# TeemoCaption/FDDM-asr

Measured on AMD Instinct MI355X. Metric: train-step utterances/sec (10 s @16 kHz, seq_len 256) at 1/2/4/8 MI355X, higher is better.
Workload: dtype bf16; 1 GPU; fddm_zhTW_base C2: WavLM-base + 6L d512 H8 ff2048 decoder, V=8000, T=200, dropout 0.1, n_step_fd=4; global_batch=32, seq_len=256, parallelism=dp1

## Files before the change

### fddm-asr_amd/csrc/norm.hip

```cpp
#include "common.h"

namespace fddm {

constexpr int LN_MAXPL = 16;

struct LnFwdArgs {
  const void* x; const void* y;
  const float *gamma, *beta, *fsc, *fsh;
  float* out_f32; void* out_t; float* save_s; float *mean, *rstd;
  long N, d, rows_per_batch;
  float eps;
  uint64_t seed, stream; unsigned thr16; float drop_scale;
  const uint64_t* seed_off;
  const float *rcos, *rsin; void* rope_out; long rope_L;
};

template <typename T>
__device__ __forceinline__ void ld8(const T* p, float (&v)[8]) {
  if constexpr (sizeof(T) == 2) {
    const uint4 u = *(const uint4*)p;
    const unsigned w[4] = {u.x, u.y, u.z, u.w};
#pragma unroll
    for (int i = 0; i < 4; ++i) {
      v[2 * i] = __uint_as_float(w[i] << 16);
      v[2 * i + 1] = __uint_as_float(w[i] & 0xffff0000u);
    }
  } else {
    const float4 a = *(const float4*)p, b = *(const float4*)(p + 4);
    v[0] = a.x; v[1] = a.y; v[2] = a.z; v[3] = a.w; v[4] = b.x; v[5] = b.y; v[6] = b.z; v[7] = b.w;
  }
}
template <typename T>
__device__ __forceinline__ void st8(T* p, const float (&v)[8]) {
  if constexpr (sizeof(T) == 2) {
    uint4 u;
    u.x = pk_bf16(v[0], v[1]);
    u.y = pk_bf16(v[2], v[3]);
    u.z = pk_bf16(v[4], v[5]);
    u.w = pk_bf16(v[6], v[7]);
    *(uint4*)p = u;
  } else {
    *(float4*)p = make_float4(v[0], v[1], v[2], v[3]);
    *(float4*)(p + 4) = make_float4(v[4], v[5], v[6], v[7]);
  }
}

template <typename OT>
__device__ __forceinline__ void st4v(OT* p, float a, float b, float c, float d_) {
  if constexpr (sizeof(OT) == 2) {
    *(uint2*)p = make_uint2(pk_bf16(a, b), pk_bf16(c, d_));
  } else {
    *(float4*)p = make_float4(a, b, c, d_);
  }
}

constexpr int LN_MAXCH = 2;

template <int CTRL>
__device__ __forceinline__ float dppf(float v) {
  return __int_as_float(__builtin_amdgcn_update_dpp(0, __float_as_int(v), CTRL, 0xF, 0xF, false));
}
__device__ __forceinline__ float wave_sum_v(float v) {
  v += dppf<0xB1>(v);
  v += dppf<0x4E>(v);
  v += dppf<0x141>(v);
  v += dppf<0x140>(v);
  auto r = __builtin_amdgcn_permlane16_swap(__float_as_uint(v), __float_as_uint(v), false, false);
  v = __uint_as_float(r[0]) + __uint_as_float(r[1]);
  r = __builtin_amdgcn_permlane32_swap(__float_as_uint(v), __float_as_uint(v), false, false);
  return __uint_as_float(r[0]) + __uint_as_float(r[1]);
}

template <typename XT, typename YT, typename OT, bool HY, bool HF, int CH, bool RP = false>
__global__ void __launch_bounds__(256) ln_fwd_kernel(LnFwdArgs a) {
  const int lane = threadIdx.x & 63;
  const long row = (long)blockIdx.x * 4 + __builtin_amdgcn_readfirstlane(threadIdx.x >> 6);
  if (row >= a.N) return;
  const long d = a.d, nch = d / 8;
  const XT* x = (const XT*)a.x + row * d;
  const YT* y = HY ? (const YT*)a.y + row * d : nullptr;
  const long b = HF ? row / a.rows_per_batch : 0;
  float v[CH][8], yv[CH][8], gm[CH][8], bt[CH][8], fs[CH][8], fh[CH][8], rc[CH][8], rs[CH][8];
  const long rp = RP ? row % a.rope_L : 0;
#pragma unroll
  for (int i = 0; i < CH; ++i) {
    const long c0 = min(lane + 64L * i, nch - 1) * 8;
    ld8<XT>(x + c0, v[i]);
    if constexpr (HY) ld8<YT>(y + c0, yv[i]);
    ld8<float>(a.gamma + c0, gm[i]);
    ld8<float>(a.beta + c0, bt[i]);
    if constexpr (HF) {
      ld8<float>(a.fsc + b * d + c0, fs[i]);
      ld8<float>(a.fsh + b * d + c0, fh[i]);
    }
    if constexpr (RP) {
      ld8<float>(a.rcos + rp * d + c0, rc[i]);
      ld8<float>(a.rsin + rp * d + c0, rs[i]);
    }
  }
  float sum = 0.f;
#pragma unroll
  for (int i = 0; i < CH; ++i) {
    const long ch = lane + 64L * i;
    if (ch >= nch) {
#pragma unroll
      for (int e = 0; e < 8; ++e) v[i][e] = 0.f;
    } else {
      if constexpr (HY) {
        unsigned keep = 0xffu;
        if (a.thr16) {
          const uint64_t e4 = (uint64_t)(row * d + ch * 8) >> 2;
          keep = drop_keep4(eff_seed(a.seed, a.seed_off), a.stream, e4, a.thr16) | (drop_keep4(eff_seed(a.seed, a.seed_off), a.stream, e4 + 1, a.thr16) << 4);
        }
#pragma unroll
        for (int e = 0; e < 8; ++e) {
          const float t = yv[i][e];
          v[i][e] += a.thr16 ? ((keep >> e) & 1u ? t * a.drop_scale : 0.f) : t;
        }
      }
#pragma unroll
      for (int e = 0; e < 8; ++e) sum += v[i][e];
    }
  }
  const float mean = wave_sum_v(sum) / (float)d;
  float sq = 0.f;
#pragma unroll
  for (int i = 0; i < CH; ++i) {
    const long ch = lane + 64L * i;
    if (ch < nch) {
#pragma unroll
      for (int e = 0; e < 8; ++e) {
        const float t = v[i][e] - mean;
        sq += t * t;
      }
    }
  }
  const float var = wave_sum_v(sq) / (float)d;
  const float rstd = 1.f / sqrtf(var + a.eps);
#pragma unroll
  for (int i = 0; i < CH; ++i) {
    const long ch = lane + 64L * i;
    if (ch < nch) {
      const long c0 = ch * 8;
      if (a.save_s) st8<float>(a.save_s + row * d + c0, v[i]);
      float o[8];
#pragma unroll
      for (int e = 0; e < 8; ++e) o[e] = (v[i][e] - mean) * rstd * gm[i][e] + bt[i][e];
      if constexpr (HF) {
#pragma unroll
        for (int e = 0; e < 8; ++e) o[e] = o[e] * (1.f + fs[i][e]) + fh[i][e];
      }
      if (a.out_f32) st8<float>(a.out_f32 + row * d + c0, o);
      if (a.out_t) st8<OT>((OT*)a.out_t + row * d + c0, o);
      if constexpr (RP) {
        float lo[4], hi[4];
#pragma unroll
        for (int j = 0; j < 4; ++j) {
          lo[j] = o[2 * j] * rc[i][2 * j] - o[2 * j + 1] * rs[i][2 * j + 1];
          hi[j] = o[2 * j] * rs[i][2 * j] + o[2 * j + 1] * rc[i][2 * j + 1];
        }
        OT* ro = (OT*)a.rope_out + row * d;
        st4v<OT>(ro + 4 * ch, lo[0], lo[1], lo[2], lo[3]);
        st4v<OT>(ro + d / 2 + 4 * ch, hi[0], hi[1], hi[2], hi[3]);
      }
    }
  }
  if (lane == 0) {
    if (a.mean) a.mean[row] = mean;
    if (a.rstd) a.rstd[row] = rstd;
  }
}

struct LnBwdArgs {
  const float* dout; const float* s; const float *mean, *rstd, *gamma, *beta, *fsc;
  float* dres; void* dy_t;
  float *dgamma, *dbeta, *dfsc, *dfsh;
  float* part;
  long N, d, rows_per_batch;
  uint64_t seed, stream; unsigned thr16; float drop_scale;
  const uint64_t* seed_off;
};

template <typename OT>
__global__ void __launch_bounds__(256) ln_bwd_kernel(LnBwdArgs a) {
// ... 300 lines not shown
    if (!(x_dtype == FDDM_F32 && y_dtype == FDDM_BF16 && out_dtype == FDDM_BF16 && hy && !hf))
      return (int)hipErrorInvalidValue;
    if (ch1) hipLaunchKernelGGL((ln_fwd_kernel<float, bf16_t, bf16_t, true, false, 1, true>), grid, dim3(256), 0, s, a);
    else hipLaunchKernelGGL((ln_fwd_kernel<float, bf16_t, bf16_t, true, false, 2, true>), grid, dim3(256), 0, s, a);
    return (int)hipGetLastError();
  }
#define LNF2(XT, YT, OT, C)                                                                                    \
  do {                                                                                                         \
    if (hy && hf) hipLaunchKernelGGL((ln_fwd_kernel<XT, YT, OT, true, true, C>), grid, dim3(256), 0, s, a);     \
    else if (hy) hipLaunchKernelGGL((ln_fwd_kernel<XT, YT, OT, true, false, C>), grid, dim3(256), 0, s, a);     \
    else if (hf) hipLaunchKernelGGL((ln_fwd_kernel<XT, YT, OT, false, true, C>), grid, dim3(256), 0, s, a);     \
    else hipLaunchKernelGGL((ln_fwd_kernel<XT, YT, OT, false, false, C>), grid, dim3(256), 0, s, a);            \
  } while (0)
#define LNF(XT, YT, OT)                \
  do {                                 \
    if (ch1) LNF2(XT, YT, OT, 1);      \
    else LNF2(XT, YT, OT, 2);          \
  } while (0)
  if (x_dtype == FDDM_F32 && y_dtype == FDDM_BF16 && out_dtype == FDDM_BF16)
    LNF(float, bf16_t, bf16_t);
  else if (x_dtype == FDDM_F32 && y_dtype == FDDM_F32 && out_dtype == FDDM_F32)
    LNF(float, float, float);
  else if (x_dtype == FDDM_BF16 && y_dtype == FDDM_BF16 && out_dtype == FDDM_BF16)
    LNF(bf16_t, bf16_t, bf16_t);
  else if (x_dtype == FDDM_F32 && y_dtype == FDDM_F32 && out_dtype == FDDM_BF16)
    LNF(float, float, bf16_t);
  else
    return (int)hipErrorInvalidValue;
#undef LNF
#undef LNF2
  return (int)hipGetLastError();
}

FDDM_API int fddm_ln_bwd(int dy_dtype, const float* dout, const float* s, const float* mean, const float* rstd,
                         const float* gamma, const float* beta, const float* film_scale, float* dres, void* dy_t,
                         float* dgamma, float* dbeta, float* dfilm_scale, float* dfilm_shift, long N, long d,
                         long rows_per_batch, float drop_p, unsigned long long seed, unsigned long long stream,
                         float* partials, void* hs) {
  if (N <= 0) return 0;
  if (d > 64 * LN_MAXPL) return (int)hipErrorInvalidValue;
  if (film_scale && (dgamma || dfilm_scale || dfilm_shift) && !(dfilm_scale && dfilm_shift))
    return (int)hipErrorInvalidValue;
  if ((dgamma == nullptr) != (dbeta == nullptr)) return (int)hipErrorInvalidValue;
  LnBwdArgs a{dout, s, mean, rstd, gamma, beta, film_scale, dres, dy_t, dgamma, dbeta, dfilm_scale, dfilm_shift,
              partials, N, d, rows_per_batch > 0 ? rows_per_batch : N, seed, stream, 0u, 1.f, g_seed_off};
  if (drop_p > 0.f) {
    a.thr16 = (unsigned)llrintf(drop_p * 65536.f);
    a.drop_scale = 1.f / (1.f - drop_p);
  }
  hipStream_t st_ = (hipStream_t)hs;
  const bool vec_ok = d % 8 == 0 && d <= 1024 &&
                      !(((uintptr_t)dout | (uintptr_t)s | (uintptr_t)gamma | (uintptr_t)beta | (uintptr_t)film_scale |
                         (uintptr_t)dres | (uintptr_t)dy_t) & 15);
  const bool fused = (dgamma || dfilm_scale) && (!film_scale || a.rows_per_batch % LNB_ROWS == 0) &&
                     (!dgamma || (beta && dbeta)) && vec_ok;
  if (partials && !dgamma) return (int)hipErrorInvalidValue;
  if (partials && !fused) {
    a.part = nullptr;
    const hipError_t e = hipMemsetAsync(partials, 0, (size_t)((N + LNB_ROWS - 1) / LNB_ROWS) * 4 * d * sizeof(float), st_);
    if (e != hipSuccess) return (int)e;
  }
  if (fused) {
    dim3 fg((unsigned)((N + LNB_ROWS - 1) / LNB_ROWS));
    const bool small = d <= 512;
    if (dy_dtype == FDDM_BF16) {
      if (small) hipLaunchKernelGGL((ln_bwd_fused_kernel<1, bf16_t>), fg, dim3(512), 0, st_, a);
// ... 43 lines not shown
```

### fddm-asr_amd/fddm_hip/functions.py

```python
from __future__ import annotations

import math
import weakref

import torch
import torch.nn.functional as F

from . import ops, runtime as rt

F32 = torch.float32


def _t(x):
    cd = rt.compute_dtype()
    return x if x.dtype == cd else ops.cast(x.contiguous(), cd)


def _gdst(p, zero=False):
    s = rt.grad_slot(p)
    if s is not None:
        return s, True
    return (torch.zeros if zero else torch.empty)(p.shape, device=p.device, dtype=F32), False


# ... 137 lines not shown
            Bt = dtb.shape[0]
            dte = torch.empty(Bt, Wp.shape[1], device=dev, dtype=F32)
            ops.small_linear(dtb, [Wp.detach()], None, [dte], transpose_w=True)
            dpre = torch.empty(Bt, W2.shape[1], device=dev, dtype=F32)
            ops.small_linear(dte, [W2.detach()], None, [dpre], act=2, aux=pre, transpose_w=True)
            ops.small_dw([(dte, h, T[2][0], T[3][0]), (dpre, emb, T[0][0], T[1][0])])
            for i in range(6):
                grads[i] = _ret(*T[i])
        return (None, None, None, None, None) + tuple(grads)


def _film_split(fs):
    return fs.contiguous()


class DecoderBlockFn(torch.autograd.Function):

    @staticmethod
    def forward(ctx, x, xT, cT, key_keep, fscale, fshift, meta, *params):
        (sa_w, sa_b, so_w, so_b, ca_w, ca_b, co_w, co_b, f0_w, f0_b, f3_w, f3_b,
         n1w, n1b, n2w, n2b, n3w, n3b) = params
        B, L, S, H, layer, p, seed, cos, sin = meta[:9]
        N, d = x.shape
        dev = x.device
        cd = rt.compute_dtype()
        st = 6 * layer
        W = {k: rt.wt(v) for k, v in (("sa", sa_w), ("so", so_w), ("ca", ca_w), ("co", co_w), ("f0", f0_w),
                                       ("f3", f3_w))}
        xr = meta[12] if len(meta) > 12 else None
        if xr is None:
            xr = torch.empty(N, d, device=dev, dtype=cd)
            ops.rope_fwd(x, cos, sin, xr, L)
        handoff = meta[13] if len(meta) > 13 else None
        qk = ops.linear(xr, W["sa"][: 2 * d], sa_b[: 2 * d], out_dtype=cd)
        v = ops.linear(xT, W["sa"][2 * d:], sa_b[2 * d:], out_dtype=cd)
        o = torch.empty(N, d, device=dev, dtype=cd)
        lse = torch.empty(B * H, L, device=dev, dtype=F32)
        pre = meta[11] if len(meta) > 11 else None
        ready = pre is not None and p > 0
        bits_s = pre[0] if ready else (ops.drop_bits(B, H, L, L, dev) if p > 0 else None)
        bits_c = pre[1] if ready else (ops.drop_bits(B, H, L, S, dev) if p > 0 else None)
        fwd_s = lambda: ops.attn_fwd(qk, qk[:, d:], v, o, lse, B, H, L, L, key_keep=key_keep, drop_p=p,
                                     seed=seed, rng_stream=st + 1, dbits=bits_s, bits_ready=ready)
        with rt.probe("decoder.self_attn_fwd", replay=fwd_s):
            fwd_s()
        y = ops.linear(o, W["so"], so_b, out_dtype=cd)
        s1 = torch.empty(N, d, device=dev, dtype=F32)
        m1 = torch.empty(N, device=dev, dtype=F32)
        r1 = torch.empty(N, device=dev, dtype=F32)
        x1 = torch.empty(N, d, device=dev, dtype=F32)
        x1T = torch.empty(N, d, device=dev, dtype=cd) if cd != F32 else x1
        ops.ln_fwd(x, y, n1w, n1b, out_f32=x1, out_t=x1T if cd != F32 else None, save_s=s1, mean=m1, rstd=r1,
                   drop_p=p, seed=seed, rng_stream=st + 2)
        qc = ops.linear(x1T, W["ca"][:d], ca_b[:d], out_dtype=cd)
        kvc = meta[10] if len(meta) > 10 and meta[10] is not None else \
            ops.linear(cT, W["ca"][d:], ca_b[d:], out_dtype=cd)
        oc = torch.empty(N, d, device=dev, dtype=cd)
        lsec = torch.empty(B * H, L, device=dev, dtype=F32)
        c_keep = meta[14] if len(meta) > 14 else None
        c_len = meta[15] if len(meta) > 15 else None
        fwd_c = lambda: ops.attn_fwd(qc, kvc, kvc[:, d:], oc, lsec, B, H, L, S, drop_p=p, seed=seed,
                                     rng_stream=st + 3, dbits=bits_c, bits_ready=ready, key_keep=c_keep,
                                     key_len=c_len)
        with rt.probe("decoder.cross_attn_fwd", replay=fwd_c):
            fwd_c()
        yc = ops.linear(oc, W["co"], co_b, out_dtype=cd)
        s2 = torch.empty(N, d, device=dev, dtype=F32)
        m2 = torch.empty(N, device=dev, dtype=F32)
        r2 = torch.empty(N, device=dev, dtype=F32)
        x2 = torch.empty(N, d, device=dev, dtype=F32)
        x2T = torch.empty(N, d, device=dev, dtype=cd) if cd != F32 else x2
        fsc, fsh = fscale.detach().contiguous(), fshift.detach().contiguous()
        ops.ln_fwd(x1, yc, n2w, n2b, out_f32=x2, out_t=x2T if cd != F32 else None, save_s=s2, mean=m2, rstd=r2,
                   film=(fsc, fsh), rows_per_batch=L, drop_p=p, seed=seed, rng_stream=st + 4)
        FF = f0_w.shape[0]
        hpre = torch.empty(N, FF, device=dev, dtype=cd)
        hact = torch.empty(N, FF, device=dev, dtype=cd)
        ops.linear(x2T, W["f0"], f0_b, out=hpre, epi=ops.EPI_GELU, C2=hact, drop_p=p, seed=seed, rng_stream=st + 5)
        y3 = ops.linear(hact, W["f3"], f3_b, out_dtype=cd)
        s3 = torch.empty(N, d, device=dev, dtype=F32)
        m3 = torch.empty(N, device=dev, dtype=F32)
        r3 = torch.empty(N, device=dev, dtype=F32)
        x3 = torch.empty(N, d, device=dev, dtype=F32)
        x3T = torch.empty(N, d, device=dev, dtype=cd)
        rope = None
        if handoff is not None and cd == torch.bfloat16 and d % 16 == 0 and d <= 1024:
            handoff["xr"] = torch.empty(N, d, device=dev, dtype=cd)
            rope = (cos, sin, handoff["xr"], L)
        ops.ln_fwd(x2, y3, n3w, n3b, out_f32=x3, out_t=x3T, save_s=s3, mean=m3, rstd=r3,
                   drop_p=p, seed=seed, rng_stream=st + 6, rope=rope)
        ctx.save_for_backward(xT, xr, qk, v, o, lse, s1, m1, r1, x1T, qc, kvc, oc, lsec, s2, m2, r2, x2T, hpre, hact,
                              s3, m3, r3, cT, key_keep, fsc, *params)
        ctx.meta = meta
        ctx.bits = (bits_s, bits_c)
        ctx.mark_non_differentiable(x3T)
        ctx.set_materialize_grads(False)
        return x3, x3T

    @staticmethod
    def backward(ctx, dx3, _dx3T):
        (xT, xr, qk, v, o, lse, s1, m1, r1, x1T, qc, kvc, oc, lsec, s2, m2, r2, x2T, hpre, hact, s3, m3, r3, cT,
         key_keep, fsc, *params) = ctx.saved_tensors
        (sa_w, sa_b, so_w, so_b, ca_w, ca_b, co_w, co_b, f0_w, f0_b, f3_w, f3_b,
         n1w, n1b, n2w, n2b, n3w, n3b) = params
        B, L, S, H, layer, p, seed, cos, sin = ctx.meta[:9]
        gfilm = ctx.meta[9] if len(ctx.meta) > 9 else None
        st = 6 * layer
        N, d = dx3.shape
        dev = dx3.device
        cd = rt.compute_dtype()
        W = {k: rt.wt(v_) for k, v_ in (("sa", sa_w), ("so", so_w), ("ca", ca_w), ("co", co_w), ("f0", f0_w),
                                         ("f3", f3_w))}
        G = [_gdst(p_, zero=True) for p_ in params]
        (gsa_w, asa), (gsa_b, _), (gso_w, aso), (gso_b, _), (gca_w, aca), (gca_b, _), (gco_w, aco), (gco_b, _), \
            (gf0_w, af0), (gf0_b, _), (gf3_w, af3), (gf3_b, _), (gn1w, _), (gn1b, _), (gn2w, _), (gn2b, _), \
            (gn3w, _), (gn3b, _) = G
        dx3 = dx3.contiguous()
        lnp = ops.LnPartials()
        dx2 = torch.empty(N, d, device=dev, dtype=F32)
        dy3 = torch.empty(N, d, device=dev, dtype=cd)
        ops.ln_bwd(dx3, s3, m3, r3, n3w, n3b, dres=dx2, dy_t=dy3, dgamma=gn3w, dbeta=gn3b, drop_p=p,
                   seed=seed, rng_stream=st + 6, partials=lnp)
        dw_jobs = [(dy3, hact, gf3_w, gf3_b)]
# ... 257 lines not shown
```

### fddm-asr_amd/fddm_hip/ops.py

```python
from __future__ import annotations

import math
import os

import torch

from ._lib import call, lib

F32, BF16 = 0, 1
EPI_STORE, EPI_GELU, EPI_ACC, EPI_GELU_ONLY, EPI_DGELU = 0, 1, 2, 3, 4


def code(t: torch.Tensor) -> int:
    if t.dtype == torch.float32:
        return F32
    if t.dtype == torch.bfloat16:
        return BF16
    raise TypeError(f"unsupported dtype {t.dtype}")


def tdtype(c: int):
    return torch.float32 if c == F32 else torch.bfloat16


# ... 320 lines not shown
def attn_bwd(q, k, v, o, do, lse, dq, dk, dv, B, H, Lq, Lk, *, key_keep=None, drop_p=0.0, seed=0, rng_stream=0,
             dbits=None, scale=None, key_len=None):
    _chk(o.shape[1] % H == 0, "attention output width must be H * head_dim")
    dh = o.shape[1] // H
    _chk(1 <= dh <= 64, f"head_dim {dh} > 64 is not built")
    if key_len is not None:
        _chk_key_len(key_len, key_keep, B, Lk)
    sc = 1.0 / math.sqrt(dh) if scale is None else scale
    if dh != 64:
        rq, rk = B * Lq, B * Lk
        dqp = torch.empty(rq, H * 64, device=dq.device, dtype=dq.dtype)
        dkp = torch.empty(rk, H * 64, device=dk.device, dtype=dk.dtype)
        dvp = torch.empty(rk, H * 64, device=dv.device, dtype=dv.dtype)
        attn_bwd(_pad64(q, rq, H, dh), _pad64(k, rk, H, dh), _pad64(v, rk, H, dh), _pad64(o, rq, H, dh),
                 _pad64(do, rq, H, dh), lse, dqp, dkp, dvp, B, H, Lq, Lk, key_keep=key_keep, drop_p=drop_p, seed=seed,
                 rng_stream=rng_stream, dbits=dbits, scale=sc)
        for g, gp, r in ((dq, dqp, rq), (dk, dkp, rk), (dv, dvp, rk)):
            _heads(g, r, H, dh).copy_(gp.view(r, H, 64)[:, :, :dh])
        return
    delta = torch.empty(int(lib().fddm_attn_bwd_ws_floats(B, H, Lq, Lk)), device=q.device, dtype=torch.float32)
    if key_len is not None:
        call("fddm_attn_bwd_kx", code(q), ptr(q), q.stride(0), ptr(k), k.stride(0), ptr(v), v.stride(0), ptr(o),
             o.stride(0), ptr(do), do.stride(0), ptr(lse), ptr(dq), dq.stride(0), ptr(dk), dk.stride(0), ptr(dv),
             dv.stride(0), ptr(delta), ptr(key_keep), ptr(key_len), B, H, Lq, Lk, float(sc), float(drop_p), seed,
             rng_stream, ptr(dbits), stream())
        return
    call("fddm_attn_bwd", code(q), ptr(q), q.stride(0), ptr(k), k.stride(0), ptr(v), v.stride(0), ptr(o),
         o.stride(0), ptr(do), do.stride(0), ptr(lse), ptr(dq), dq.stride(0), ptr(dk), dk.stride(0), ptr(dv),
         dv.stride(0), ptr(delta), ptr(key_keep), B, H, Lq, Lk, float(sc), float(drop_p), seed, rng_stream,
         ptr(dbits), stream())


def ln_fwd(x, y, gamma, beta, *, out_f32=None, out_t=None, save_s=None, mean=None, rstd=None, film=None,
           rows_per_batch=0, eps=1e-5, drop_p=0.0, seed=0, rng_stream=0, rope=None):
    N, d = x.shape
    fs, fh = film if film is not None else (None, None)
    rc, rs, ro, rl = rope if rope is not None else (None, None, None, 0)
    out_code = code(out_t) if out_t is not None else code(x if y is None else y)
    ycode = code(y) if y is not None else code(x)
    call("fddm_ln_fwd", code(x), ycode, out_code, ptr(x), ptr(y), ptr(gamma), ptr(beta), ptr(fs), ptr(fh),
         ptr(out_f32), ptr(out_t), ptr(save_s), ptr(mean), ptr(rstd), N, d, rows_per_batch, float(eps), float(drop_p),
         seed, rng_stream, ptr(rc), ptr(rs), ptr(ro), rl, stream())


def ln_bwd(dout, s, mean, rstd, gamma, beta, *, dres=None, dy_t=None, dgamma=None, dbeta=None, film_scale=None,
           dfilm=None, rows_per_batch=0, drop_p=0.0, seed=0, rng_stream=0, partials=None):
    N, d = dout.shape
    dfs, dfh = dfilm if dfilm is not None else (None, None)
    part = None
    if partials is not None:
        _chk(dgamma is not None and dbeta is not None, "ln_bwd partials need dgamma and dbeta")
        part = partials.add(N, d, dgamma, dbeta, (dfs, dfh) if film_scale is not None else None, rows_per_batch)
    call("fddm_ln_bwd", code(dy_t) if dy_t is not None else F32, ptr(dout), ptr(s), ptr(mean), ptr(rstd), ptr(gamma),
         ptr(beta), ptr(film_scale), ptr(dres), ptr(dy_t), ptr(dgamma), ptr(dbeta), ptr(dfs), ptr(dfh), N, d,
         rows_per_batch, float(drop_p), seed, rng_stream, ptr(part), stream())


class LnPartials:

    def __init__(self):
        self.jobs = []

    def add(self, N, d, dgamma, dbeta, dfilm=None, rows_per_batch=0):
        _chk(len(self.jobs) < 4, "at most 4 LayerNorms per fold")
        rows = lib().fddm_ln_bwd_slab_rows()
        nslab = (N + rows - 1) // rows
        part = torch.empty(nslab, 4, d, device=dgamma.device, dtype=torch.float32)
        dfs = dfh = None
        spb = 0
        if dfilm is not None and rows_per_batch > 0 and rows_per_batch % rows == 0:
            dfs, dfh = dfilm
            spb = rows_per_batch // rows
        self.jobs.append((part, nslab, d, dgamma, dbeta, dfs, dfh, spb))
        return part

# ... 302 lines not shown
```

### fddm-asr_amd/fddm_hip/runtime.py

```python
from __future__ import annotations

import contextlib
import math
import os

import weakref

import torch

from . import ops

_precision = os.environ.get("FDDM_PRECISION", "bf16")


def precision() -> str:
    return _precision


def set_precision(p: str) -> None:
    global _precision
    if p not in ("bf16", "fp32"):
        raise ValueError(p)
    _precision = p


@contextlib.contextmanager
def use_precision(p: str):
    old = _precision
    set_precision(p)
    try:
        yield
    finally:
        set_precision(old)


def compute_dtype():
    return torch.bfloat16 if _precision == "bf16" else torch.float32


class _Entry:
    __slots__ = ("version", "tensor", "ptr", "ref")

    def valid_for(self, p) -> bool:
        return self.ref() is p and self.version == p._version and self.ptr == p.data_ptr()


def _entry(p, tensor) -> _Entry:
    e = _Entry()
    e.version, e.tensor, e.ptr, e.ref = p._version, tensor, p.data_ptr(), weakref.ref(p)
    return e


_wcache: dict = {}
_wcache_gen = 0
_cache_epoch = 0
_retained = None


def cache_epoch() -> int:
    return _cache_epoch


@contextlib.contextmanager
def retaining():
    global _retained
    old, _retained = _retained, []
    try:
        yield _retained
    finally:
        if old is not None:
# ... 244 lines not shown
```

### fddm-asr_amd/models/denoise_decoder.py

```python
from __future__ import annotations

import math
from typing import Literal, Optional, Tuple

import torch
import torch.nn as nn
import torch.nn.functional as F

from fddm_hip import functions as FN
from fddm_hip import runtime as rt
from fddm_hip.ops import attn_drop_bits as ops_attn_drop_bits
from fddm_hip.ops import drop_words
from fddm_hip.ops import linear as ops_linear
from fddm_hip.ops import key_extent as ops_key_extent
from fddm_hip.ops import rows_mean as ops_rows_mean
from fddm_hip.ops import rows_mean_masked as ops_rows_mean_masked


class RoPEEmbedding(nn.Module):

    def __init__(self, d_model: int, base: float = 10000.0):
        super().__init__()
        self.d_model = d_model
        self.base = base
# ... 53 lines not shown
        self.out_proj = nn.Linear(d_model, d_model)
        nn.init.xavier_uniform_(self.in_proj_weight)
        nn.init.zeros_(self.out_proj.bias)


class DecoderBlock(nn.Module):

    def __init__(self, d_model: int, nhead: int, dim_ff: int, dropout: float = 0.1, use_film: bool = True,
                 pos_emb_type: str = "rope"):
        super().__init__()
        if pos_emb_type != "rope" or not use_film:
            raise NotImplementedError("only the reference's default block (rope + FiLM) is built")
        if d_model % nhead or d_model // nhead > 64:
            raise NotImplementedError("head_dim = d_model / nhead must divide d_model and be <= 64 on this build")
        self.use_film, self.pos_emb_type = use_film, pos_emb_type
        self.nhead, self.p = nhead, dropout
        self.self_attn = _MHAParams(d_model, nhead, dropout)
        self.cross_attn = _MHAParams(d_model, nhead, dropout)
        self.film_layer = FiLMLayer(d_model, d_model)
        self.ff = nn.Sequential(nn.Linear(d_model, dim_ff), nn.GELU(), nn.Dropout(dropout), nn.Linear(dim_ff, d_model))
        self.norm1 = nn.LayerNorm(d_model)
        self.norm2 = nn.LayerNorm(d_model)
        self.norm3 = nn.LayerNorm(d_model)
        self.drop = nn.Dropout(dropout)

    def block_params(self):
        return (self.self_attn.in_proj_weight, self.self_attn.in_proj_bias, self.self_attn.out_proj.weight,
                self.self_attn.out_proj.bias, self.cross_attn.in_proj_weight, self.cross_attn.in_proj_bias,
                self.cross_attn.out_proj.weight, self.cross_attn.out_proj.bias, self.ff[0].weight, self.ff[0].bias,
                self.ff[3].weight, self.ff[3].bias, self.norm1.weight, self.norm1.bias, self.norm2.weight,
                self.norm2.bias, self.norm3.weight, self.norm3.bias)

    def run(self, x, xT, cT, key_keep, film, B, L, S, layer, seed, cos, sin, kv=None, bits=None, xr=None,
            handoff=None, c_keep=None, c_len=None):
        fscale, fshift, gfilm = film
        p = self.p if self.training else 0.0
        meta = (B, L, S, self.nhead, layer, p, seed, cos, sin, gfilm, kv, bits, xr, handoff, c_keep, c_len)
        return FN.DecoderBlockFn.apply(x, xT, cT, key_keep, fscale, fshift, meta, *self.block_params())


class DenoisingTransformerDecoder(nn.Module):

    def __init__(self, vocab_size: int, d_model: int = 768, nhead: int = 12, num_layers: int = 6, dim_ff: int = 2048,
                 dropout: float = 0.1, max_len: int = 2048, pad_id: int = 0,
                 pos_emb_type: Literal["rope", "sinusoidal", "learned"] = "rope", use_film: bool = True,
                 rope_base: float = 10000.0) -> None:
        super().__init__()
        if pos_emb_type != "rope":
            raise NotImplementedError("pos_emb_type != 'rope' is out of scope (train.py always uses rope)")
        self.pos_emb_type, self.use_film = pos_emb_type, use_film
        self.tok_emb = nn.Embedding(vocab_size, d_model, padding_idx=pad_id)
        self.pos_emb = RoPEEmbedding(d_model, base=rope_base)
        self.time_emb = SinusoidalTimeEmbedding(d_model)
        self.time_proj = nn.Linear(d_model, d_model)
        self.blocks = nn.ModuleList([DecoderBlock(d_model, nhead, dim_ff, dropout, use_film, pos_emb_type)
                                     for _ in range(num_layers)])
        self.head = nn.Linear(d_model, vocab_size)
        self.pad_id = pad_id
        self.d_model, self.nhead = d_model, nhead

    def forward(self, xt: torch.Tensor, t: torch.Tensor, cond: torch.Tensor, x_mask: Optional[torch.Tensor] = None,
                c_mask: Optional[torch.Tensor] = None) -> torch.Tensor:
        B, L = xt.shape
        S = cond.shape[1]
        dev = xt.device
        cd = rt.compute_dtype()
        c_keep = c_len = None
        with torch.no_grad():
            cc = cond.detach()
            cc = cc if cc.is_contiguous() else cc.contiguous()
            if c_mask is None:
                pooled = ops_rows_mean(cc)
            else:
                c_keep = c_mask.to(dev)
                c_keep = c_keep.contiguous().view(torch.uint8) if c_keep.dtype == torch.bool else \
                    (c_keep != 0).contiguous().view(torch.uint8)
                c_len = ops_key_extent(c_keep)
                pooled = ops_rows_mean_masked(cc, c_keep, clamp=False)
        nb = len(self.blocks)
        gbuf = torch.zeros(2 * nb, B, self.d_model, device=dev, dtype=torch.float32)
        te = self.time_emb
        film_params = [q for blk in self.blocks for lin in (blk.film_layer.scale_proj, blk.film_layer.shift_proj)
                       for q in (lin.weight, lin.bias)]
        outs = FN.CondFn.apply(t, pooled, gbuf, self.d_model, te.max_steps, te.mlp[0].weight, te.mlp[0].bias,
                               te.mlp[2].weight, te.mlp[2].bias, self.time_proj.weight, self.time_proj.bias,
                               *film_params)
        t_bias, films = outs[0], outs[1:]
        if t_bias.shape[0] != B:
            t_bias = t_bias.expand(B, -1)
        x, xT = FN.EmbedFn.apply(xt, self.tok_emb.weight, t_bias, self.pad_id)
        if x_mask is None:
            x_mask = xt != self.pad_id
        key_keep = x_mask.contiguous().view(torch.uint8) if x_mask.dtype == torch.bool else \
            x_mask.to(torch.uint8).contiguous()
        with torch.no_grad():
            c = cond.detach()
            cT = (c if c.dtype == cd else c.to(cd)).reshape(B * S, -1).contiguous()
        cos, sin = self.pos_emb(L, dev)
        seed = rt.next_seed()
        kv_all = self._cross_kv(cT)
        bits = self._drop_bits(B, L, S, seed, dev)
        xr = None
        for i, blk in enumerate(self.blocks):
            film = (films[2 * i], films[2 * i + 1], (gbuf[2 * i], gbuf[2 * i + 1]))
            kv = None if kv_all is None else kv_all[:, 2 * self.d_model * i: 2 * self.d_model * (i + 1)]
            bi = None if bits is None else (bits[0][i], bits[1][i])
            handoff = {} if i + 1 < len(self.blocks) else None
            x, xT = blk.run(x, xT, cT, key_keep, film, B, L, S, i, seed, cos, sin, kv, bi, xr, handoff, c_keep,
                            c_len)
            xr = None if handoff is None else handoff.get("xr")
        logits = FN.HeadFn.apply(x, xT, self.head.weight, self.head.bias)
        return logits.view(B, L, -1)

    @torch.no_grad()
    def _drop_bits(self, B, L, S, seed, dev):
        p = self.blocks[0].p if (self.training and len(self.blocks)) else 0.0
        if p <= 0 or rt.compute_dtype() != torch.bfloat16:
            return None
        H, nb = self.nhead, len(self.blocks)
        ws = drop_words(B, H, L, L)
        wc = drop_words(B, H, L, S)
        bs = torch.empty(nb, ws, device=dev, dtype=torch.int64)
        bc = torch.empty(nb, wc, device=dev, dtype=torch.int64)
        ops_attn_drop_bits(bs, nb, B, H, L, L, p, seed, 1, 6)
        ops_attn_drop_bits(bc, nb, B, H, L, S, p, seed, 3, 6)
        return bs, bc

    @torch.no_grad()
    def _cross_kv(self, cT):
        if len(self.blocks) < 2:
            return None
        d = self.d_model
        w = torch.cat([rt.wt(blk.cross_attn.in_proj_weight)[d:] for blk in self.blocks])
        b = torch.cat([blk.cross_attn.in_proj_bias.detach()[d:] for blk in self.blocks])
        return ops_linear(cT, w, b, out_dtype=rt.compute_dtype())

    def grad_ready_order(self):
        out = [self.head.weight, self.head.bias]
        for blk in reversed(self.blocks):
            out += [p for n, p in blk.named_parameters() if not n.startswith("film_layer.")]
        seen = set(id(p) for p in out)
        return out + [p for p in self.parameters() if id(p) not in seen]

# ... 4 lines not shown
```

### include/fddm_hip.h

```cpp
#ifndef FDDM_HIP_H
#define FDDM_HIP_H
#ifdef __cplusplus
extern "C" {
#endif

int fddm_abi_version(void);
const char* fddm_error_string(int code);

int fddm_gemm(int dtype, int a_dtype, int a_kc, int b_kc, int epi, int out_dtype, const void* A, long lda, long Mi,
              long sAb, const void* B, long ldb, void* C, long ldc, void* C2, const float* bias, float alpha, long M,
              long N, long K, unsigned long long seed, unsigned long long stream, float drop_p, float* colsum,
              void* hip_stream);

int fddm_linear_dx_rope(const void* dy, long ldy, const void* w, long ldw, float* dx, long lddx, const float* cs,
                        const float* sn, long M, long N, long K, long L, void* hip_stream);

int fddm_gemm_persistent_cap(int cap);

int fddm_gemm_dw_grouped(int n, const void* const* dy, const long* ldy, const void* const* x, const long* ldx,
                         float* const* dw, const long* lddw, float* const* db, const long* M, const long* N,
                         const long* K, long kchunk, void* hip_stream);

int fddm_conv1d_gemm(int dtype, int epi, const void* x, long lda, long sAb, long Tin, long Cg, long cstride,
                     long cpad, const void* W, void* out, long ldc, const float* bias, long Bn, long Tout, long N,
// ... 20 lines not shown
int fddm_attn_fwd_relgate(const void* Q, long sq, const void* K, long sk, const void* V, long sv, void* O, long so,
                          const void* graw, long sgr, const float* gconst, const float* table, int B, int H, int Lq,
                          int Lk, float scale, void* hip_stream);
int fddm_attn_fwd_relgate_x(const void* Q, long sq, const void* K, long sk, const void* V, long sv, void* O, long so,
                            const void* x, long sx, const float* gw, const float* gconst, const float* table, int B,
                            int H, int Lq, int Lk, float scale, void* hip_stream);
long fddm_attn_bwd_ws_floats(int B, int H, int Lq, int Lk);
int fddm_attn_bwd(int dtype, const void* Q, long sq, const void* K, long sk, const void* V, long sv, const void* O,
                  long so, const void* dO, long sdo, const float* lse, void* dQ, long sdq, void* dK, long sdk,
                  void* dV, long sdv, float* delta_ws, const unsigned char* key_keep, int B, int H, int Lq, int Lk,
                  float scale, float drop_p, unsigned long long seed, unsigned long long stream,
                  const unsigned long long* drop_bits, void* hip_stream);

int fddm_attn_fwd_kx(int dtype, const void* Q, long sq, const void* K, long sk, const void* V, long sv, void* O,
                     long so, float* lse, const unsigned char* key_keep, const int* key_len, const float* gate,
                     const float* table, int B, int H, int Lq, int Lk, float scale, float drop_p,
                     unsigned long long seed, unsigned long long stream, unsigned long long* drop_bits,
                     int drop_bits_ready, void* hip_stream);
int fddm_attn_bwd_kx(int dtype, const void* Q, long sq, const void* K, long sk, const void* V, long sv, const void* O,
                     long so, const void* dO, long sdo, const float* lse, void* dQ, long sdq, void* dK, long sdk,
                     void* dV, long sdv, float* delta_ws, const unsigned char* key_keep, const int* key_len, int B,
                     int H, int Lq, int Lk, float scale, float drop_p, unsigned long long seed,
                     unsigned long long stream, const unsigned long long* drop_bits, void* hip_stream);
int fddm_attn_fwd_relgate_x_kx(const void* Q, long sq, const void* K, long sk, const void* V, long sv, void* O,
                               long so, const void* x, long sx, const float* gw, const float* gconst,
                               const float* table, const unsigned char* key_keep, const int* key_len, int B, int H,
                               int Lq, int Lk, float scale, void* hip_stream);

int fddm_ln_fwd(int x_dtype, int y_dtype, int out_dtype, const void* x, const void* y, const float* gamma,
                const float* beta, const float* film_scale, const float* film_shift, float* out_f32, void* out_t,
                float* save_s, float* mean, float* rstd, long N, long d, long rows_per_batch, float eps, float drop_p,
                unsigned long long seed, unsigned long long stream, const float* rope_cos, const float* rope_sin,
                void* rope_out, long rope_L, void* hip_stream);
int fddm_ln_bwd(int dy_dtype, const float* dout, const float* s, const float* mean, const float* rstd,
                const float* gamma, const float* beta, const float* film_scale, float* dres, void* dy_t,
                float* dgamma, float* dbeta, float* dfilm_scale, float* dfilm_shift, long N, long d,
                long rows_per_batch, float drop_p, unsigned long long seed, unsigned long long stream,
                float* partials, void* hip_stream);
int fddm_ln_bwd_slab_rows(void);
int fddm_ln_fold(int n, const float* const* partials, const long* nslab, const long* d, float* const* dgamma,
                 float* const* dbeta, float* const* dfilm_scale, float* const* dfilm_shift,
                 const long* slabs_per_batch, void* hip_stream);

int fddm_rope_fwd(int out_dtype, const float* x, const float* cs, const float* sn, void* out, long N, long L, long d,
                  void* hip_stream);
int fddm_rope_bwd(const float* dy, const float* cs, const float* sn, float* dx, long N, long L, long d,
                  void* hip_stream);

int fddm_embed_fwd(int out_dtype, const long* tok, const float* E, const float* tbias, float* out, void* out_t, long N,
                   long L, long d, void* hip_stream);
int fddm_embed_bwd(const long* tok, const float* dx, float* dE, float* dtb, long N, long L, long d, long pad_id,
                   void* hip_stream);

int fddm_colsum(int dtype, const void* X, float* out, long M, long N, long ldx, void* hip_stream);
int fddm_cast(int src_dtype, int dst_dtype, const void* x, void* y, long n, void* hip_stream);

int fddm_sample_q(const long* x0, const long* t, const unsigned* thr, long* xt, long B, long L, long K,
                  unsigned long long seed, unsigned long long stream, void* hip_stream);
int fddm_kl_fwd(const float* logits, const long* xt, const long* x0, const long* t, const float* betas, float* kl_tok,
                long N, long L, long V, void* hip_stream);
int fddm_kl_bwd(const float* logits, const long* xt, const long* x0, const long* t, const float* betas,
                const float* w, const float* gscale, void* dz, int dz_dtype, long N, long L, long V,
                void* hip_stream);
int fddm_kl_fused(const float* logits, const long* xt, const long* x0, const long* t, const float* betas,
                  const unsigned char* mask, float* kl_tok, void* dz, int dz_dtype, long N, long L, long V,
                  void* hip_stream);
// ... 61 lines not shown
```

Measured before the change: 3372 utterances/s.

## Recompute previous LayerNorm output in next LN instead of storing fp32 activations

Adds a chained LayerNorm forward kernel that rebuilds the previous LN's output from its saved pre-norm sum, mean, rstd, gamma/beta and optional FiLM. The fp32 out_f32 tensors for the decoder's post-attention, cross-attention and FFN norms, including the hand-off to the next block, no longer need to be written and read back. This trades one fp32 N×d store and load per LN for extra parameter loads and arithmetic, and adds considerable plumbing plus an env toggle that is on by default.

```diff
diff --git a/fddm-asr_amd/csrc/norm.hip b/fddm-asr_amd/csrc/norm.hip
--- a/fddm-asr_amd/csrc/norm.hip
+++ b/fddm-asr_amd/csrc/norm.hip
@@ -13,7 +13,16 @@
   uint64_t seed, stream; unsigned thr16; float drop_scale;
   const uint64_t* seed_off;
   const float *rcos, *rsin; void* rope_out; long rope_L;
+  const float *s_p, *mean_p, *rstd_p, *gamma_p, *beta_p, *fsc_p, *fsh_p;
+  long rpb_p;
 };
+
+template <bool FILM>
+__device__ __forceinline__ float ln_affine(float s, float mean, float rstd, float g, float b, float fs, float fh) {
+  float o = fmaf((s - mean) * rstd, g, b);
+  if constexpr (FILM) o = fmaf(o, 1.f + fs, fh);
+  return o;
+}
 
 template <typename T>
 __device__ __forceinline__ void ld8(const T* p, float (&v)[8]) {
@@ -71,21 +80,40 @@
   return __uint_as_float(r[0]) + __uint_as_float(r[1]);
 }
 
-template <typename XT, typename YT, typename OT, bool HY, bool HF, int CH, bool RP = false>
+template <typename XT, typename YT, typename OT, bool HY, bool HF, int CH, bool RP = false, bool CN = false,
+          bool PF = false>
 __global__ void __launch_bounds__(256) ln_fwd_kernel(LnFwdArgs a) {
   const int lane = threadIdx.x & 63;
   const long row = (long)blockIdx.x * 4 + __builtin_amdgcn_readfirstlane(threadIdx.x >> 6);
   if (row >= a.N) return;
   const long d = a.d, nch = d / 8;
-  const XT* x = (const XT*)a.x + row * d;
+  const XT* x = CN ? nullptr : (const XT*)a.x + row * d;
+  const float* sp = CN ? a.s_p + row * d : nullptr;
+  const long pb_ = PF ? row / a.rpb_p : 0;
+  float pmean = 0.f, prstd = 0.f;
+  if constexpr (CN) {
+    pmean = a.mean_p[row];
+    prstd = a.rstd_p[row];
+  }
   const YT* y = HY ? (const YT*)a.y + row * d : nullptr;
   const long b = HF ? row / a.rows_per_batch : 0;
   float v[CH][8], yv[CH][8], gm[CH][8], bt[CH][8], fs[CH][8], fh[CH][8], rc[CH][8], rs[CH][8];
+  float pg[CH][8], pbt[CH][8], pfs[CH][8], pfh[CH][8];
   const long rp = RP ? row % a.rope_L : 0;
 #pragma unroll
   for (int i = 0; i < CH; ++i) {
     const long c0 = min(lane + 64L * i, nch - 1) * 8;
-    ld8<XT>(x + c0, v[i]);
+    if constexpr (CN) {
+      ld8<float>(sp + c0, v[i]);
+      ld8<float>(a.gamma_p + c0, pg[i]);
+      ld8<float>(a.beta_p + c0, pbt[i]);
+      if constexpr (PF) {
+        ld8<float>(a.fsc_p + pb_ * d + c0, pfs[i]);
+        ld8<float>(a.fsh_p + pb_ * d + c0, pfh[i]);
+      }
+    } else {
+      ld8<XT>(x + c0, v[i]);
+    }
     if constexpr (HY) ld8<YT>(y + c0, yv[i]);
     ld8<float>(a.gamma + c0, gm[i]);
     ld8<float>(a.beta + c0, bt[i]);
@@ -106,6 +134,11 @@
 #pragma unroll
       for (int e = 0; e < 8; ++e) v[i][e] = 0.f;
     } else {
+      if constexpr (CN) {
+#pragma unroll
+        for (int e = 0; e < 8; ++e)
+          v[i][e] = ln_affine<PF>(v[i][e], pmean, prstd, pg[i][e], pbt[i][e], PF ? pfs[i][e] : 0.f, PF ? pfh[i][e] : 0.f);
+      }
       if constexpr (HY) {
         unsigned keep = 0xffu;
         if (a.thr16) {
@@ -145,11 +178,8 @@
       if (a.save_s) st8<float>(a.save_s + row * d + c0, v[i]);
       float o[8];
 #pragma unroll
-      for (int e = 0; e < 8; ++e) o[e] = (v[i][e] - mean) * rstd * gm[i][e] + bt[i][e];
-      if constexpr (HF) {
-#pragma unroll
-        for (int e = 0; e < 8; ++e) o[e] = o[e] * (1.f + fs[i][e]) + fh[i][e];
-      }
+      for (int e = 0; e < 8; ++e)
+        o[e] = ln_affine<HF>(v[i][e], mean, rstd, gm[i][e], bt[i][e], HF ? fs[i][e] : 0.f, HF ? fh[i][e] : 0.f);
       if (a.out_f32) st8<float>(a.out_f32 + row * d + c0, o);
       if (a.out_t) st8<OT>((OT*)a.out_t + row * d + c0, o);
       if constexpr (RP) {
@@ -516,6 +546,59 @@
   return (int)hipGetLastError();
 }
 
+FDDM_API int fddm_ln_fwd_chain(const float* s_prev, const float* mean_prev, const float* rstd_prev,
+                               const float* gamma_prev, const float* beta_prev, const float* film_scale_prev,
+                               const float* film_shift_prev, long rows_per_batch_prev, const void* y,
+                               const float* gamma, const float* beta, const float* film_scale,
+                               const float* film_shift, float* out_f32, void* out_t, float* save_s, float* mean,
+                               float* rstd, long N, long d, long rows_per_batch, float eps, float drop_p,
+                               unsigned long long seed, unsigned long long stream, const float* rope_cos,
+                               const float* rope_sin, void* rope_out, long rope_L, void* hs) {
+  if (N <= 0) return 0;
+  if (d > 64 * 8 * LN_MAXCH || d % 8) return (int)hipErrorInvalidValue;
+  if (!s_prev || !mean_prev || !rstd_prev || !gamma_prev || !beta_prev || !y || !gamma || !beta)
+    return (int)hipErrorInvalidValue;
+  if ((film_scale == nullptr) != (film_shift == nullptr) || (film_scale_prev == nullptr) != (film_shift_prev == nullptr))
+    return (int)hipErrorInvalidValue;
+  if (rope_out && (film_scale || !rope_cos || !rope_sin || rope_L <= 0 || d % 16 ||
+                   (((uintptr_t)rope_cos | (uintptr_t)rope_sin | (uintptr_t)rope_out) & 15)))
+    return (int)hipErrorInvalidValue;
+  if ((((uintptr_t)gamma | (uintptr_t)beta | (uintptr_t)film_scale | (uintptr_t)film_shift | (uintptr_t)y |
+        (uintptr_t)s_prev | (uintptr_t)gamma_prev | (uintptr_t)beta_prev | (uintptr_t)film_scale_prev |
+        (uintptr_t)film_shift_prev | (uintptr_t)out_f32 | (uintptr_t)out_t | (uintptr_t)save_s) & 15))
+    return (int)hipErrorInvalidValue;
+  LnFwdArgs a{nullptr, y, gamma, beta, film_scale, film_shift, out_f32, out_t, save_s, mean, rstd, N, d,
+              rows_per_batch > 0 ? rows_per_batch : N, eps, seed, stream, 0u, 1.f, g_seed_off, rope_cos, rope_sin,
+              rope_out, rope_L, s_prev, mean_prev, rstd_prev, gamma_prev, beta_prev, film_scale_prev, film_shift_prev,
+              rows_per_batch_prev > 0 ? rows_per_batch_prev : N};
+  if (drop_p > 0.f) {
+    a.thr16 = (unsigned)llrintf(drop_p * 65536.f);
+    a.drop_scale = 1.f / (1.f - drop_p);
+  }
+  dim3 grid((unsigned)((N + 3) / 4));
+  hipStream_t s = (hipStream_t)hs;
+  const bool hf = film_scale != nullptr, rp = rope_out != nullptr, pf = film_scale_prev != nullptr;
+#define LNC3(HF_, C, RP_, PF_) \
+  hipLaunchKernelGGL((ln_fwd_kernel<float, bf16_t, bf16_t, true, HF_, C, RP_, true, PF_>), grid, dim3(256), 0, s, a)
+#define LNC2(C, PF_)                        \
+  do {                                      \
+    if (hf) LNC3(true, C, false, PF_);      \
+    else if (rp) LNC3(false, C, true, PF_); \
+    else LNC3(false, C, false, PF_);        \
+  } while (0)
+#define LNC(C)               \
+  do {                       \
+    if (pf) LNC2(C, true);   \
+    else LNC2(C, false);     \
+  } while (0)
+  if (d <= 512) LNC(1);
+  else LNC(2);
+#undef LNC
+#undef LNC2
+#undef LNC3
+  return (int)hipGetLastError();
+}
+
 FDDM_API int fddm_ln_bwd(int dy_dtype, const float* dout, const float* s, const float* mean, const float* rstd,
                          const float* gamma, const float* beta, const float* film_scale, float* dres, void* dy_t,
                          float* dgamma, float* dbeta, float* dfilm_scale, float* dfilm_shift, long N, long d,
diff --git a/fddm-asr_amd/fddm_hip/functions.py b/fddm-asr_amd/fddm_hip/functions.py
--- a/fddm-asr_amd/fddm_hip/functions.py
+++ b/fddm-asr_amd/fddm_hip/functions.py
@@ -193,6 +193,9 @@
             xr = torch.empty(N, d, device=dev, dtype=cd)
             ops.rope_fwd(x, cos, sin, xr, L)
         handoff = meta[13] if len(meta) > 13 else None
+        chain = bool(meta[16]) if len(meta) > 16 else False
+        lnp = meta[17] if len(meta) > 17 else None
+        fuse = chain and cd == torch.bfloat16 and d % 8 == 0 and d <= 1024
         qk = ops.linear(xr, W["sa"][: 2 * d], sa_b[: 2 * d], out_dtype=cd)
         v = ops.linear(xT, W["sa"][2 * d:], sa_b[2 * d:], out_dtype=cd)
         o = torch.empty(N, d, device=dev, dtype=cd)
@@ -209,10 +212,11 @@
         s1 = torch.empty(N, d, device=dev, dtype=F32)
         m1 = torch.empty(N, device=dev, dtype=F32)
         r1 = torch.empty(N, device=dev, dtype=F32)
-        x1 = torch.empty(N, d, device=dev, dtype=F32)
+        x1 = None if fuse else torch.empty(N, d, device=dev, dtype=F32)
         x1T = torch.empty(N, d, device=dev, dtype=cd) if cd != F32 else x1
-        ops.ln_fwd(x, y, n1w, n1b, out_f32=x1, out_t=x1T if cd != F32 else None, save_s=s1, mean=m1, rstd=r1,
-                   drop_p=p, seed=seed, rng_stream=st + 2)
+        ops.ln_fwd(x if lnp is None else None, y, n1w, n1b, out_f32=x1, out_t=x1T if cd != F32 else None, save_s=s1,
+                   mean=m1, rstd=r1, drop_p=p, seed=seed, rng_stream=st + 2,
+                   prev=None if lnp is None else (*lnp, None, 0))
         qc = ops.linear(x1T, W["ca"][:d], ca_b[:d], out_dtype=cd)
         kvc = meta[10] if len(meta) > 10 and meta[10] is not None else \
             ops.linear(cT, W["ca"][d:], ca_b[d:], out_dtype=cd)
@@ -229,11 +233,12 @@
         s2 = torch.empty(N, d, device=dev, dtype=F32)
         m2 = torch.empty(N, device=dev, dtype=F32)
         r2 = torch.empty(N, device=dev, dtype=F32)
-        x2 = torch.empty(N, d, device=dev, dtype=F32)
+        x2 = None if fuse else torch.empty(N, d, device=dev, dtype=F32)
         x2T = torch.empty(N, d, device=dev, dtype=cd) if cd != F32 else x2
         fsc, fsh = fscale.detach().contiguous(), fshift.detach().contiguous()
         ops.ln_fwd(x1, yc, n2w, n2b, out_f32=x2, out_t=x2T if cd != F32 else None, save_s=s2, mean=m2, rstd=r2,
-                   film=(fsc, fsh), rows_per_batch=L, drop_p=p, seed=seed, rng_stream=st + 4)
+                   film=(fsc, fsh), rows_per_batch=L, drop_p=p, seed=seed, rng_stream=st + 4,
+                   prev=(s1, m1, r1, n1w, n1b, None, 0) if fuse else None)
         FF = f0_w.shape[0]
         hpre = torch.empty(N, FF, device=dev, dtype=cd)
         hact = torch.empty(N, FF, device=dev, dtype=cd)
@@ -242,14 +247,18 @@
         s3 = torch.empty(N, d, device=dev, dtype=F32)
         m3 = torch.empty(N, device=dev, dtype=F32)
         r3 = torch.empty(N, device=dev, dtype=F32)
-        x3 = torch.empty(N, d, device=dev, dtype=F32)
         x3T = torch.empty(N, d, device=dev, dtype=cd)
         rope = None
         if handoff is not None and cd == torch.bfloat16 and d % 16 == 0 and d <= 1024:
             handoff["xr"] = torch.empty(N, d, device=dev, dtype=cd)
             rope = (cos, sin, handoff["xr"], L)
-        ops.ln_fwd(x2, y3, n3w, n3b, out_f32=x3, out_t=x3T, save_s=s3, mean=m3, rstd=r3,
-                   drop_p=p, seed=seed, rng_stream=st + 6, rope=rope)
+        carry = fuse and (handoff is None or rope is not None)
+        x3 = s3 if carry else torch.empty(N, d, device=dev, dtype=F32)
+        if carry and handoff is not None:
+            handoff["ln"] = (s3, m3, r3, n3w.detach(), n3b.detach())
+        ops.ln_fwd(x2, y3, n3w, n3b, out_f32=None if carry else x3, out_t=x3T, save_s=s3, mean=m3, rstd=r3,
+                   drop_p=p, seed=seed, rng_stream=st + 6, rope=rope,
+                   prev=(s2, m2, r2, n2w, n2b, (fsc, fsh), L) if fuse else None)
         ctx.save_for_backward(xT, xr, qk, v, o, lse, s1, m1, r1, x1T, qc, kvc, oc, lsec, s2, m2, r2, x2T, hpre, hact,
                               s3, m3, r3, cT, key_keep, fsc, *params)
         ctx.meta = meta
diff --git a/fddm-asr_amd/fddm_hip/ops.py b/fddm-asr_amd/fddm_hip/ops.py
--- a/fddm-asr_amd/fddm_hip/ops.py
+++ b/fddm-asr_amd/fddm_hip/ops.py
@@ -376,7 +376,10 @@
 
 
 def ln_fwd(x, y, gamma, beta, *, out_f32=None, out_t=None, save_s=None, mean=None, rstd=None, film=None,
-           rows_per_batch=0, eps=1e-5, drop_p=0.0, seed=0, rng_stream=0, rope=None):
+           rows_per_batch=0, eps=1e-5, drop_p=0.0, seed=0, rng_stream=0, rope=None, prev=None):
+    if prev is not None:
+        return _ln_fwd_chain(prev, x, y, gamma, beta, out_f32, out_t, save_s, mean, rstd, film, rows_per_batch, eps,
+                             drop_p, seed, rng_stream, rope)
     N, d = x.shape
     fs, fh = film if film is not None else (None, None)
     rc, rs, ro, rl = rope if rope is not None else (None, None, None, 0)
@@ -385,6 +388,59 @@
     call("fddm_ln_fwd", code(x), ycode, out_code, ptr(x), ptr(y), ptr(gamma), ptr(beta), ptr(fs), ptr(fh),
          ptr(out_f32), ptr(out_t), ptr(save_s), ptr(mean), ptr(rstd), N, d, rows_per_batch, float(eps), float(drop_p),
          seed, rng_stream, ptr(rc), ptr(rs), ptr(ro), rl, stream())
+
+
+def _ln_operand(t, name, dtype, shape):
+    _chk(t.dtype == dtype, f"ln_fwd chain: {name} must be {dtype}, got {t.dtype}")
+    _chk(tuple(t.shape) == tuple(shape), f"ln_fwd chain: {name} must be {tuple(shape)}, got {tuple(t.shape)}")
+    _chk(t.is_contiguous(), f"ln_fwd chain: {name} must be contiguous")
+
+
+def _ln_fwd_chain(prev, x, y, gamma, beta, out_f32, out_t, save_s, mean, rstd, film, rows_per_batch, eps, drop_p,
+                  seed, rng_stream, rope):
+    f32, bf16 = torch.float32, torch.bfloat16
+    _chk(len(prev) == 7, "ln_fwd chain: prev = (s, mean, rstd, gamma, beta, film_or_None, rows_per_batch)")
+    sp, mp, rp, gp, bp, fp, rpb_p = prev
+    _chk(sp.dim() == 2, "ln_fwd chain: s_prev must be [N, d]")
+    N, d = sp.shape
+    _chk(d % 8 == 0 and 0 < d <= 1024, f"ln_fwd chain: d % 8 == 0 and d <= 1024 required, got d = {d}")
+    _ln_operand(sp, "s_prev", f32, (N, d))
+    _ln_operand(mp, "mean_prev", f32, (N,))
+    _ln_operand(rp, "rstd_prev", f32, (N,))
+    _ln_operand(gp, "gamma_prev", f32, (d,))
+    _ln_operand(bp, "beta_prev", f32, (d,))
+    fsp = fhp = None
+    rpb_p = int(rpb_p)
+    if fp is not None:
+        fsp, fhp = fp
+        _chk(rpb_p > 0 and N % rpb_p == 0, "ln_fwd chain: previous FiLM needs rows_per_batch dividing N")
+        _ln_operand(fsp, "film_scale_prev", f32, (N // rpb_p, d))
+        _ln_operand(fhp, "film_shift_prev", f32, (N // rpb_p, d))
+    _chk(x is None or tuple(x.shape) == (N, d), f"ln_fwd chain: x is {tuple(x.shape) if x is not None else None}, "
+                                                f"s_prev {(N, d)}")
+    _chk(y is not None, "ln_fwd chain: the residual branch y is required")
+    _ln_operand(y, "y", bf16, (N, d))
+    _ln_operand(gamma, "gamma", f32, (d,))
+    _ln_operand(beta, "beta", f32, (d,))
+    fs = fh = None
+    if film is not None:
+        fs, fh = film
+        _chk(rows_per_batch > 0 and N % rows_per_batch == 0, "ln_fwd chain: FiLM needs rows_per_batch dividing N")
+        _ln_operand(fs, "film_scale", f32, (N // rows_per_batch, d))
+        _ln_operand(fh, "film_shift", f32, (N // rows_per_batch, d))
+    for t, name, dt, shp in ((out_f32, "out_f32", f32, (N, d)), (out_t, "out_t", bf16, (N, d)),
+                             (save_s, "save_s", f32, (N, d)), (mean, "mean", f32, (N,)), (rstd, "rstd", f32, (N,))):
+        if t is not None:
+            _ln_operand(t, name, dt, shp)
+    rc, rs, ro, rl = rope if rope is not None else (None, None, None, 0)
+    if rope is not None:
+        _chk(film is None and d % 16 == 0 and rl > 0, "ln_fwd chain: rope needs d % 16 == 0, L > 0 and no FiLM")
+        _ln_operand(rc, "rope cos", f32, (rl, d))
+        _ln_operand(rs, "rope sin", f32, (rl, d))
+        _ln_operand(ro, "rope out", bf16, (N, d))
+    call("fddm_ln_fwd_chain", ptr(sp), ptr(mp), ptr(rp), ptr(gp), ptr(bp), ptr(fsp), ptr(fhp), rpb_p, ptr(y),
+         ptr(gamma), ptr(beta), ptr(fs), ptr(fh), ptr(out_f32), ptr(out_t), ptr(save_s), ptr(mean), ptr(rstd), N, d,
+         rows_per_batch, float(eps), float(drop_p), seed, rng_stream, ptr(rc), ptr(rs), ptr(ro), rl, stream())
 
 
 def ln_bwd(dout, s, mean, rstd, gamma, beta, *, dres=None, dy_t=None, dgamma=None, dbeta=None, film_scale=None,
diff --git a/fddm-asr_amd/fddm_hip/runtime.py b/fddm-asr_amd/fddm_hip/runtime.py
--- a/fddm-asr_amd/fddm_hip/runtime.py
+++ b/fddm-asr_amd/fddm_hip/runtime.py
@@ -36,6 +36,18 @@
 
 def compute_dtype():
     return torch.bfloat16 if _precision == "bf16" else torch.float32
+
+
+_ln_chain = os.environ.get("FDDM_LN_CHAIN", "1") != "0"
+
+
+def ln_chain() -> bool:
+    return _ln_chain
+
+
+def set_ln_chain(on: bool) -> None:
+    global _ln_chain
+    _ln_chain = bool(on)
 
 
 class _Entry:
diff --git a/fddm-asr_amd/models/denoise_decoder.py b/fddm-asr_amd/models/denoise_decoder.py
--- a/fddm-asr_amd/models/denoise_decoder.py
+++ b/fddm-asr_amd/models/denoise_decoder.py
@@ -109,10 +109,11 @@
                 self.norm2.bias, self.norm3.weight, self.norm3.bias)
 
     def run(self, x, xT, cT, key_keep, film, B, L, S, layer, seed, cos, sin, kv=None, bits=None, xr=None,
-            handoff=None, c_keep=None, c_len=None):
+            handoff=None, c_keep=None, c_len=None, chain=False, ln_prev=None):
         fscale, fshift, gfilm = film
         p = self.p if self.training else 0.0
-        meta = (B, L, S, self.nhead, layer, p, seed, cos, sin, gfilm, kv, bits, xr, handoff, c_keep, c_len)
+        meta = (B, L, S, self.nhead, layer, p, seed, cos, sin, gfilm, kv, bits, xr, handoff, c_keep, c_len, chain,
+                ln_prev)
         return FN.DecoderBlockFn.apply(x, xT, cT, key_keep, fscale, fshift, meta, *self.block_params())
 
 
@@ -177,15 +178,17 @@
         seed = rt.next_seed()
         kv_all = self._cross_kv(cT)
         bits = self._drop_bits(B, L, S, seed, dev)
-        xr = None
+        chain = rt.ln_chain() and cd == torch.bfloat16
+        xr = ln_prev = None
         for i, blk in enumerate(self.blocks):
             film = (films[2 * i], films[2 * i + 1], (gbuf[2 * i], gbuf[2 * i + 1]))
             kv = None if kv_all is None else kv_all[:, 2 * self.d_model * i: 2 * self.d_model * (i + 1)]
             bi = None if bits is None else (bits[0][i], bits[1][i])
             handoff = {} if i + 1 < len(self.blocks) else None
             x, xT = blk.run(x, xT, cT, key_keep, film, B, L, S, i, seed, cos, sin, kv, bi, xr, handoff, c_keep,
-                            c_len)
+                            c_len, chain, ln_prev)
             xr = None if handoff is None else handoff.get("xr")
+            ln_prev = None if handoff is None else handoff.get("ln")
         logits = FN.HeadFn.apply(x, xT, self.head.weight, self.head.bias)
         return logits.view(B, L, -1)
 
diff --git a/include/fddm_hip.h b/include/fddm_hip.h
--- a/include/fddm_hip.h
+++ b/include/fddm_hip.h
@@ -76,6 +76,13 @@
                 float* save_s, float* mean, float* rstd, long N, long d, long rows_per_batch, float eps, float drop_p,
                 unsigned long long seed, unsigned long long stream, const float* rope_cos, const float* rope_sin,
                 void* rope_out, long rope_L, void* hip_stream);
+int fddm_ln_fwd_chain(const float* s_prev, const float* mean_prev, const float* rstd_prev, const float* gamma_prev,
+                      const float* beta_prev, const float* film_scale_prev, const float* film_shift_prev,
+                      long rows_per_batch_prev, const void* y, const float* gamma, const float* beta,
+                      const float* film_scale, const float* film_shift, float* out_f32, void* out_t, float* save_s,
+                      float* mean, float* rstd, long N, long d, long rows_per_batch, float eps, float drop_p,
+                      unsigned long long seed, unsigned long long stream, const float* rope_cos,
+                      const float* rope_sin, void* rope_out, long rope_L, void* hip_stream);
 int fddm_ln_bwd(int dy_dtype, const float* dout, const float* s, const float* mean, const float* rstd,
                 const float* gamma, const float* beta, const float* film_scale, float* dres, void* dy_t,
                 float* dgamma, float* dbeta, float* dfilm_scale, float* dfilm_shift, long N, long d,
```

Measured after the change: 3365 utterances/s. Within noise of the previous version (-0.2%).
